# taleinat/fuzzysearch

Hardware: NVIDIA H100
Metric: haystack_GB_per_s_scanned (higher is better)
Workload: dtype u8

## Files before the change

### fuzzysearch_b200/csrc/api.cu

```cuda
#include <algorithm>
#include <atomic>
#include <cstdarg>
#include <cstdio>
#include <cmath>
#include <cstring>
#include <dlfcn.h>
#include <sched.h>
#include <unistd.h>
#include <condition_variable>
#include <memory>
#include <mutex>
#include <thread>
#include <new>
#include <string>
#include <type_traits>
#include <vector>

#include "kernels.cuh"
#include "ham_kernels.cuh"
#include "lp_kernels.cuh"
#include "post_kernels.cuh"
#include "p2p_kernels.cuh"
#include "batch_kernels.cuh"
#include "ham_batch_kernels.cuh"
#include "generic_batch_kernels.cuh"
#include "best_kernels.cuh"
#include "nearest_kernels.cuh"
#include "sym_kernels.cuh"
#include "align_kernels.cuh"
#include <unordered_map>
#include "debug_kernels.cuh"

using namespace fzb;

static thread_local std::string g_err;

static int fail(int code, const char *fmt, ...) {
    char buf[512];
    va_list ap;
    va_start(ap, fmt);
    vsnprintf(buf, sizeof buf, fmt, ap);
    va_end(ap);
    g_err = buf;
    return code;
// ... 54 lines not shown
    T *p_ = nullptr;
    uint64_t n_ = 0;
};
template <class T> using DevBuf = Buf<T, Mem::Device>;
template <class T> using PinnedBuf = Buf<T, Mem::Pinned>;
template <class T> using MappedBuf = Buf<T, Mem::Mapped>;

struct BatchBufs {
    DevBuf<uint32_t> d_mbits;
    DevBuf<uint2> d_gtab;
    DevBuf<uint32_t> d_postings, d_pinfo;
    DevBuf<BatchPat> d_bpats;
    DevBuf<unsigned long long> d_mset;
    DevBuf<WorkItem> d_mwork;
};
struct LpBatchBufs {
    DevBuf<ulonglong2> d_lmlut;
    DevBuf<unsigned long long> d_lmlist;
    DevBuf<unsigned long long> d_lmkept;
    DevBuf<uint32_t> d_lmhist;
};
struct GenericBatchBufs {
    DevBuf<uint32_t> d_glim;
};
struct PeerBufs {
    DevBuf<uint8_t> d_p2p;
    DevBuf<MergeScratch> d_ms;
    DevBuf<unsigned long long> d_mscore;
    DevBuf<uint32_t> d_mpos;
    MappedBuf<int64_t> h_grows;
    MappedBuf<uint32_t> h_ghdr;
};
struct RecBufs {
    DevBuf<uint64_t> d_off;
    DevBuf<uint32_t> d_first;
    uint64_t longest = 0;
};
struct BestBufs {
    DevBuf<uint64_t> d_words;
    DevBuf<uint32_t> d_ids;
};
struct BestState {
    uint64_t *best, *top2;
    const uint32_t *ordinal;
};
struct NearBufs {
// ... 108 lines not shown
    uint32_t p2p_cap = 4096;
    uint64_t slot_bytes = 0, flags_off = 0;
    uint32_t epoch = 0;
    bool counters_clean = false;
    uint32_t seq = 0;
    void *comm = nullptr;
    int rank = 0, world = 1;
    uint32_t gather_cap = 4096;
    std::unique_ptr<GatherBufs> gather;
    cudaEvent_t ev[4] = {nullptr, nullptr, nullptr, nullptr};
    int sm_count = 132;
    DevBuf<uint64_t> d_hits;
    DevBuf<uint32_t> d_glist;
    uint32_t glist_cap = 0;
    DevBuf<uint32_t> d_scratch;
    DevBuf<unsigned long long> d_lplist;
    std::unique_ptr<BatchBufs> batch;
    DevBuf<unsigned long long> d_mhits;
    std::unique_ptr<LpBatchBufs> lpb;
    std::unique_ptr<GenericBatchBufs> gbatch;
    std::unique_ptr<RecBufs> recs;
    std::unique_ptr<BestBufs> bestb;
    std::unique_ptr<NearBufs> nearb;
};

struct fzb_result {
    std::vector<RawRec> raw;
    uint32_t raw_n = 0;
    fzb_haystack *owner = nullptr;
    bool raw_in_stage = false;
    void fetch_raw();
    void discard_attempt();
    std::vector<RawRec> fin;
    std::vector<int64_t> hulls;
    bool unconsolidated = false;
    bool have_fin = false;
    bool device_post = false;
    bool raw_ordered = false;
    bool has_global = false;
    bool global_on_device = false;
    bool fused_issued = false;
    uint32_t fused_status = 0;
    uint32_t gcount = 0;
    std::vector<RawRec> gfin;
    int raw_order = 0;
    void order_raw();
    fzb_stats stats{};
};

static uint64_t round_up(uint64_t x, uint64_t a) { return (x + a - 1) / a * a; }

static RawRec make_rec(int64_t start, int64_t end, int64_t dist) {
    RawRec r;
    r.start = start;
// ... 5 lines not shown
}

struct HandleLock {
    std::recursive_mutex *m;
    explicit HandleLock(fzb_haystack *h) : m(h ? &h->mu : nullptr) {
        if (m) m->lock();
    }
    ~HandleLock() {
        if (m) m->unlock();
    }
    HandleLock(const HandleLock &) = delete;
    HandleLock &operator=(const HandleLock &) = delete;
};

static std::mutex g_pending_mutex;

void fzb_result::fetch_raw() {
    std::lock_guard<std::mutex> lock(g_pending_mutex);
    if (!owner) return;
    if (raw_in_stage) {
        raw.resize(raw_n);
        if (raw_n) {
            cudaSetDevice(owner->device);
            if (cudaMemcpyAsync(raw.data(), owner->d_out.get(), (size_t)raw_n * sizeof(RawRec), cudaMemcpyDeviceToHost,
                                owner->stream) != cudaSuccess ||
                cudaStreamSynchronize(owner->stream) != cudaSuccess) {
                cudaGetLastError();
                raw.clear();
                raw_n = 0;
            }
        }
        raw_in_stage = false;
    }
    if (global_on_device) {
        gfin.resize(gcount);
        for (uint32_t i = 0; i < gcount; i++) {
            const int64_t s0 = owner->peer->h_grows[2 * (size_t)i], v = owner->peer->h_grows[2 * (size_t)i + 1];
            gfin[i] = make_rec(s0, s0 + (v >> 32), v & 0xFFFFFFFF);
        }
        global_on_device = false;
    }
    owner->pending = nullptr;
    owner = nullptr;
}

void fzb_result::discard_attempt() {
    fetch_raw();
    raw.clear();
    raw_n = 0;
    fin.clear();
}

static void detach_pending(fzb_haystack *h) {
    fzb_result *r;
    {
        std::lock_guard<std::mutex> lock(g_pending_mutex);
        r = h->pending;
    }
    if (r) r->fetch_raw();
}

static int alloc_out(fzb_haystack *h, uint64_t cap) { return h->d_out.alloc(cap, cap * (sizeof(RawRec) + sizeof(uint64_t))); }

static int haystack_common_init(fzb_haystack *h) {
    CK(cudaSetDevice(h->device));
    CK(cudaStreamCreateWithFlags(&h->stream, cudaStreamNonBlocking));
    for (auto &e : h->ev) CK(cudaEventCreate(&e));
    CK(cudaEventCreate(&h->ev_stop));
    cudaDeviceProp prop;
    CK(cudaGetDeviceProperties(&prop, h->device));
    h->sm_count = prop.multiProcessorCount;
    uint64_t granules = (h->padded_len >> kGranuleShift) + 2;
    TRY(h->d_bitmap.alloc(round_up((granules + 31) / 32, 32)));
    TRY(h->d_counters.alloc(CNT_COUNT));
    TRY(h->h_counters.alloc(CNT_COUNT));
    memset(h->h_counters.get(), 0, CNT_COUNT * sizeof(uint32_t));
    TRY(h->h_fin.alloc((uint64_t)kPostMax * kFinCols));
    TRY(h->d_fin.alloc((uint64_t)kPostMax * kFinCols));
    TRY(h->d_sorted.alloc(kPostMax));
    CK(cudaFuncSetAttribute(k_post, cudaFuncAttributeMaxDynamicSharedMemorySize, (int)kPostSmem));
    CK(cudaMemset(h->d_bitmap.get(), 0, h->d_bitmap.size() * sizeof(uint32_t)));
    h->glist_cap = (uint32_t)std::min<uint64_t>(granules, 1u << 20);
    TRY(h->d_glist.alloc(std::max<uint32_t>(h->glist_cap, 1)));
    return alloc_out(h, 1u << 16);
}

static int check_shard(uint64_t buf_len, uint64_t buf_lo, uint64_t global_len, uint64_t own_lo,
                       uint64_t own_hi) {
    if (global_len >= (1ull << 46)) return fail(FZB_E_INVALID, "global_len must be below 2^46");
    if (buf_lo > global_len || buf_len > global_len - buf_lo || own_lo > own_hi || own_hi > global_len ||
        (own_lo < own_hi && (own_lo < buf_lo || own_hi > buf_lo + buf_len)))
        return fail(FZB_E_INVALID, "inconsistent shard geometry");
    if (buf_lo % 16 != 0) return fail(FZB_E_INVALID, "buf_lo must be a multiple of 16");
    if (buf_len >= (1ull << 40)) return fail(FZB_E_INVALID, "buf_len must be below 2^40");
    return FZB_OK;
}

static int alloc_buffer(fzb_haystack *h) {
    CK(cudaSetDevice(h->device));
    TRY(h->owned_buf.alloc(h->padded_len));
    h->d = h->owned_buf.get();
    CK(cudaMemset(h->d + h->buf_len, 0, h->padded_len - h->buf_len));
    return FZB_OK;
}

static void close_peers(fzb_haystack *h);
static int upload_bytes(fzb_haystack *h, uint64_t dst_off, const uint8_t *host, uint64_t n);

extern "C" void fzb_haystack_destroy(fzb_haystack *h) {
    if (!h) return;
    cudaSetDevice(h->device);
    if (h->stream) cudaStreamSynchronize(h->stream);
    detach_pending(h);
    if (h->comm) nccl_comm_destroy(h->comm);
    close_peers(h);
    for (auto &e : h->ev)
        if (e) cudaEventDestroy(e);
    if (h->ev_stop) cudaEventDestroy(h->ev_stop);
    if (h->stream) cudaStreamDestroy(h->stream);
    delete h;
}

static int haystack_new(const char *arg_error, const uint8_t *host, const void *dev_ptr, uint64_t buf_len,
                        uint64_t buf_lo, uint64_t global_len, uint64_t own_lo, uint64_t own_hi, int device,
                        fzb_haystack **out) {
    if (!out) return fail(FZB_E_INVALID, "out is NULL");
    *out = nullptr;
    if (arg_error) return fail(FZB_E_INVALID, "%s", arg_error);
    int rc = check_shard(buf_len, buf_lo, global_len, own_lo, own_hi);
    if (rc) return rc;
    if (fzb_device_count() <= device || device < 0)
        return fail(FZB_E_CUDA, "CUDA device %d not available (%d devices)", device, fzb_device_count());
    fzb_haystack *h = new (std::nothrow) fzb_haystack();
    if (!h) return fail(FZB_E_CUDA, "out of host memory");
    h->device = device;
    h->d = (uint8_t *)dev_ptr;
// ... 1454 lines not shown
        TRY(b.d_bpats.alloc(kMaxBatchPats));
        TRY(b.d_mset.alloc(1u << 22));
        CK(cudaMemset(b.d_mset.get(), 0, b.d_mset.size() * sizeof(unsigned long long)));
        TRY(b.d_mwork.alloc(1u << 21));
        CK(cudaFuncSetAttribute(k_filter_multi, cudaFuncAttributeMaxDynamicSharedMemorySize, (int)kMultiSmem));
        return FZB_OK;
    });
}

static int read_counters(fzb_haystack *h, uint32_t cnts[CNT_COUNT]) {
    CK(cudaMemcpyAsync(cnts, h->d_counters.get(), CNT_COUNT * sizeof(uint32_t), cudaMemcpyDeviceToHost, h->stream));
    CK(cudaStreamSynchronize(h->stream));
    return FZB_OK;
}

static void add_stats(fzb_stats *sum, const fzb_stats &s) {
    sum->gpu_ms += s.gpu_ms;
    sum->filter_ms += s.filter_ms;
    sum->bytes_scanned += s.bytes_scanned;
    sum->n_candidates += s.n_candidates;
    sum->n_launches += s.n_launches;
}

static int split_batch(const std::vector<RawRec> &raw, const std::vector<uint32_t> &ids, const fzb_stats &pass,
                       int raw_order, bool unconsolidated, fzb_result **out, fzb_stats *sum) {
    const uint32_t cnt = (uint32_t)ids.size();
    std::vector<uint32_t> per(cnt, 0);
    for (const RawRec &r : raw) per[(uint32_t)r.ngram >> 8]++;
    for (uint32_t i = 0; i < cnt; i++) {
        fzb_result *res = new (std::nothrow) fzb_result();
        if (!res) return fail(FZB_E_CUDA, "out of host memory");
        res->raw.reserve(per[i]);
        if (i == 0) res->stats = pass;
        res->stats.route = pass.route;
        res->raw_order = raw_order;
        out[ids[i]] = res;
    }
    for (const RawRec &r : raw) {
        RawRec q = r;
        q.ngram = r.ngram & 0xFF;
        out[ids[(uint32_t)r.ngram >> 8]]->raw.push_back(q);
    }
    const unsigned nthreads = std::min<unsigned>({8u, std::max(1u, std::thread::hardware_concurrency()), cnt});
    std::atomic<uint32_t> next{0};
    auto work = [&]() {
        for (uint32_t i = next.fetch_add(1); i < cnt; i = next.fetch_add(1)) {
            fzb_result *res = out[ids[i]];
            res->raw_n = (uint32_t)res->raw.size();
            res->unconsolidated = unconsolidated;
            if (unconsolidated)
                finalize_on_host(res, 2);
            else
                consolidate_recs(res->raw, res->fin, &res->hulls);
            res->have_fin = true;
        }
    };
    std::vector<std::thread> pool;
    for (unsigned t = 1; t < nthreads; t++) pool.emplace_back(work);
    work();
    for (auto &t : pool) t.join();
    add_stats(sum, pass);
    return FZB_OK;
}

static int best_accumulate(fzb_haystack *h, const BestState &best, uint32_t n, const uint32_t *d_ids, uint32_t id) {
    if (n == 0) return FZB_OK;
    const int grid = (int)std::min<uint32_t>((n + kBestThreads - 1) / kBestThreads, (uint32_t)h->sm_count * 8);
    if (d_ids)
        k_best_accumulate<true><<<grid, kBestThreads, 0, h->stream>>>(h->d_out.get(), n, rec_set(h), d_ids, id,
                                                                     best.best, best.top2);
    else
        k_best_accumulate<false><<<grid, kBestThreads, 0, h->stream>>>(h->d_out.get(), n, rec_set(h), d_ids, id,
                                                                      best.best, best.top2);
    CK(cudaGetLastError());
    return FZB_OK;
}

struct BatchCall {
    fzb_haystack *h;
    const uint8_t *patterns;
    const uint32_t *offsets;
    uint32_t count, flags;
    std::vector<Plan> plans;
    fzb_result **out;
    const BestState *best;
    std::vector<uint8_t> done;
    bool tiny, share;
    fzb_stats sum{};

    BatchCall(fzb_haystack *h_, const uint8_t *p, const uint32_t *o, uint32_t n, uint32_t f, fzb_result **out_,
              const BestState *best_)
        : h(h_), patterns(p), offsets(o), count(n), flags(f), out(out_), best(best_), done(best_ ? n : 0, 0),
          tiny((f & FZB_F_TINY_LIST) != 0), share((f & ~(FZB_F_TINY_LIST | FZB_F_PER_RECORD)) == 0 && h_->buf_len > 0) {}

    uint32_t len(uint32_t i) const { return offsets[i + 1] - offsets[i]; }
    bool settled(uint32_t i) const { return best ? done[i] != 0 : out[i] != nullptr; }

    template <class P>
    int begin(P plan) {
        for (uint32_t i = 0; i < count; i++) out[i] = nullptr;
        TRY(check_batch_records(h, flags));
        for (uint32_t i = 0; i < count; i++)
            if (offsets[i + 1] < offsets[i]) return fail(FZB_E_INVALID, "offsets must be non-decreasing");
        plans.resize(count);
        for (uint32_t i = 0; i < count; i++) TRY(plan(i, patterns + offsets[i], len(i), plans[i]));
        return FZB_OK;
    }

    int settle(int rc, const std::vector<uint32_t> &ids) {
        auto drop = [&](uint32_t j) {
            if (!out) return;
            fzb_result_destroy(out[j]);
            out[j] = nullptr;
        };
        if (rc < 0)
            for (uint32_t j = 0; j < count; j++) drop(j);
        if (rc > 0)
            for (uint32_t id : ids) drop(id);
        return rc < 0 ? rc : FZB_OK;
    }

    int finish_pass(const std::vector<RawRec> &raw, uint32_t n, const std::vector<uint32_t> &ids, fzb_stats pass,
                    int raw_order, bool unconsolidated) {
        if (!best) return split_batch(raw, ids, pass, raw_order, unconsolidated, out, &sum);
        if (n) {
            std::vector<uint32_t> ordinals(ids.size());
            for (size_t j = 0; j < ids.size(); j++) ordinals[j] = best->ordinal[ids[j]];
            CK(cudaMemcpyAsync(h->bestb->d_ids.get(), ordinals.data(), ordinals.size() * sizeof(uint32_t),
                               cudaMemcpyHostToDevice, h->stream));
            TRY(best_accumulate(h, *best, n, h->bestb->d_ids.get(), 0));
            pass.n_launches++;
        }
        for (uint32_t id : ids) done[id] = 1;
        add_stats(&sum, pass);
        return FZB_OK;
    }

    int finish(fzb_stats *total) {
        const uint32_t f = (flags & ~FZB_F_PER_RECORD) | (best ? FZB_F_NO_FINAL : 0u);
        for (uint32_t i = 0; i < count; i++) {
            if (settled(i)) continue;
            fzb_result *res = nullptr;
            auto planned = [&](Plan &pl) { pl = plans[i]; return FZB_OK; };
            TRY(settle(run_search(h, patterns + offsets[i], f, &res, planned), {}));
            if (!best) {
                add_stats(&sum, res->stats);
                out[i] = res;
                continue;
            }
            const int rc = best_accumulate(h, *best, res->raw_n, nullptr, best->ordinal[i]);
            if (res->raw_n) res->stats.n_launches++;
            add_stats(&sum, res->stats);
            fzb_result_destroy(res);
            TRY(rc);
        }
        sum.route = 7;
        if (total) *total = sum;
        return FZB_OK;
    }
};

template <class F>
static int run_batch_pass(const BatchCall &c, F enqueue, std::vector<RawRec> &raw, uint32_t cnts[CNT_COUNT],
                          fzb_stats &pass) {
    fzb_haystack *h = c.h;
    detach_pending(h);
    for (int attempt = 0; attempt < 8; attempt++) {
        h->counters_clean = false;
        CK(cudaMemsetAsync(h->d_counters.get(), 0, CNT_COUNT * sizeof(uint32_t), h->stream));
        CK(cudaEventRecord(h->ev[0], h->stream));
        int rc = enqueue();
        if (rc) return rc;
        CK(cudaEventRecord(h->ev[2], h->stream));
        rc = read_counters(h, cnts);
        if (rc) return rc;
        if (cnts[CNT_OVERFLOW]) return 1;
        const uint32_t n = cnts[CNT_OUT];
        if (n > kMaxRawRecs) return 1;
        if (n > h->d_out.size()) {
            TRY(ensure_out_cap(h, n));
            continue;
        }
        if (!c.best) raw.resize(n);
        if (!raw.empty()) {
            CK(cudaMemcpyAsync(raw.data(), h->d_out.get(), (size_t)n * sizeof(RawRec), cudaMemcpyDeviceToHost, h->stream));
            CK(cudaStreamSynchronize(h->stream));
        }
        float ms = 0.f;
        cudaEventElapsedTime(&ms, h->ev[0], h->ev[2]);
        pass.gpu_ms = ms;
        pass.bytes_scanned = h->buf_len;
        return FZB_OK;
    }
    return fail(FZB_E_CUDA, "output buffer kept overflowing");
}

struct ChunkSums {
    float scan_ms = 0.f;
    uint64_t listed = 0;
    uint32_t chunks = 0;
};

template <class S, class V>
static int run_chunks(fzb_haystack *h, uint64_t chunk, int list, int full, uint32_t cnts[CNT_COUNT], ChunkSums &s,
                      S scan, V verify) {
    s = ChunkSums{};
    for (uint64_t lo = h->own_lo; lo < h->own_hi; lo += chunk) {
        CK(cudaMemsetAsync(h->d_counters.get() + list, 0, 2 * sizeof(uint32_t), h->stream));
        CK(cudaEventRecord(h->ev[1], h->stream));
// ... 136 lines not shown
    std::vector<uint32_t> bits(kMultiTblWords + (dense ? 0 : kMulti2Words), 0);
    int rc = upload_pass_tables(h, grams, bits, pinfo, pats, [&](uint32_t w) {
        const uint32_t hb = (w * kHashMul) >> (32 - kMultiTblBits);
        bits[hb >> 5] |= 1u << (hb & 31u);
        if (!dense) {
            const uint32_t h2 = multi_hash2(w);
            bits[kMultiTblWords + (h2 >> 5)] |= 1u << (h2 & 31u);
        }
    });
    if (rc) return rc;
    if (dense) TRY(ensure_mhits(h));
    const int ggrid = h->sm_count * 4;
    if (generic) TRY(prepare_generic_pass(c, ids, ggrid));
    BatchBufs &b = *h->batch;
    MultiParams mp = pass_params(h);
    mp.bits2 = dense ? nullptr : b.d_mbits.get() + kMultiTblWords;
    mp.set = b.d_mset.get();
    mp.set_mask = (uint32_t)b.d_mset.size() - 1;
    mp.work = b.d_mwork.get();
    mp.work_cap = c.tiny ? std::min<uint32_t>(b.d_mwork.size(), kTinyBatchCap) : (uint32_t)b.d_mwork.size();
    const uint32_t hits_cap = c.tiny ? std::min<uint32_t>(h->d_mhits.size(), kTinyBatchCap) : (uint32_t)h->d_mhits.size();
    const int64_t nvec = (int64_t)(round_up(h->buf_len, 16) / 16);
    const int64_t ntiles = (nvec + kMultiTileVecs - 1) / kMultiTileVecs;
    std::vector<RawRec> raw;
    uint32_t cnts[CNT_COUNT];
    fzb_stats pass{};
    const RecSet rs = rec_set(h);
    rc = run_batch_pass(c, [&]() -> int {
        MdenseParams dp{mp, b.d_bpats.get(), h->d_mhits.get(), hits_cap};
        if (ntiles > 0) {
            const int grid = (int)std::min<int64_t>(ntiles, h->sm_count);
            if (dense)
                k_filter_mdense<<<grid, kMultiThreads, kMdenseSmem, h->stream>>>(dp, nvec, ntiles);
            else
                k_filter_multi<<<grid, kMultiThreads, kMultiSmem, h->stream>>>(mp, nvec, ntiles);
        }
        CK(cudaEventRecord(h->ev[1], h->stream));
        with_recs(h, [&](auto rec) {
            constexpr bool R = decltype(rec)::value;
            if (generic && dense)
                k_verify_mhits_generic<R><<<ggrid, kLpThreads, 0, h->stream>>>(
                    dp, h->gbatch->d_glim.get(), h->d_scratch.get(), kGenericBatchCap, h->d_out.get(), h->d_out.size(),
                    h->d_counters.get(), rs);
            else if (generic)
                k_verify_multi_generic<R><<<ggrid, kLpThreads, 0, h->stream>>>(
                    mp, b.d_bpats.get(), h->gbatch->d_glim.get(), h->d_scratch.get(), kGenericBatchCap, h->d_out.get(),
                    h->d_out.size(), h->d_counters.get(), rs);
            else if (dense)
                k_verify_mhits<R><<<h->sm_count * 8, kMhThreads, 0, h->stream>>>(dp, h->d_out.get(), h->d_out.size(),
                                                                                    h->d_counters.get(), rs);
            else
                k_verify_multi<R><<<h->sm_count * 8, kVmThreads, 0, h->stream>>>(
                    mp, b.d_bpats.get(), h->d_out.get(), h->d_out.size(), h->d_counters.get(), rs);
        });
        CK(cudaGetLastError());
        return FZB_OK;
    }, raw, cnts, pass);
    if (rc > 0 && !dense) {
        CK(cudaMemsetAsync(b.d_mset.get(), 0, b.d_mset.size() * sizeof(unsigned long long), h->stream));
        CK(cudaStreamSynchronize(h->stream));
    }
    if (rc) return rc;
    float filter_ms = 0.f;
    cudaEventElapsedTime(&filter_ms, h->ev[0], h->ev[1]);
    pass.route = generic ? 9 : dense ? 2 : 1;
    pass.filter_ms = filter_ms;
    pass.n_candidates = cnts[CNT_CAND];
    pass.n_launches = 2;
    return c.finish_pass(raw, cnts[CNT_OUT], ids, pass, generic ? 2 : 0, false);
}

static int batch_pass_lp(BatchCall &c, const std::vector<uint32_t> &ids) {
    fzb_haystack *h = c.h;
    const uint32_t cnt = (uint32_t)ids.size();
    const bool generic = c.plans[ids[0]].generic();
    std::vector<BatchPat> pats(cnt);
    std::vector<ulonglong2> lut(256, make_ulonglong2(0ull, 0ull));
    std::vector<uint32_t> pm32((size_t)cnt * 256, 0u);
    LpMultiParams lp{};
    int wmax = 0;
    uint32_t kmax = 0;
    for (uint32_t i = 0; i < cnt; i++) {
        const uint32_t id = ids[i], m = c.len(id), k = c.plans[id].k;
        BatchPat &bp = pats[i];
        fill_pat(bp, c, id);
        for (uint32_t j = 0; j < m; j++) {
            lut[bp.P[j]].x |= 1ull << i;
            pm32[(size_t)i * 256 + bp.P[j]] |= 1u << j;
        }
        if (generic)
            for (int c = 0; c < 256; c++) lut[c].y |= 1ull << i;
        else
// ... 19 lines not shown
    uint32_t *d_pm32 = reinterpret_cast<uint32_t *>(lb.d_lmlut.get() + 256);
    CK(cudaMemcpyAsync(d_pm32, pm32.data(), pm32.size() * sizeof(uint32_t), cudaMemcpyHostToDevice, h->stream));
    CK(cudaMemcpyAsync(h->batch->d_bpats.get(), pats.data(), pats.size() * sizeof(BatchPat), cudaMemcpyHostToDevice, h->stream));
    lp.H = h->d;
    lp.buf_lo = (int64_t)h->buf_lo;
    lp.buf_len = (int64_t)h->buf_len;
    lp.N = (int64_t)h->global_len;
    lp.lut = lb.d_lmlut.get();
    lp.wmax = wmax;
    lp.pats = h->batch->d_bpats.get();
    lp.pm32 = d_pm32;
    lp.list = lb.d_lmlist.get();
    lp.list_cap = c.tiny ? std::min<uint32_t>(lb.d_lmlist.size(), kTinyLpListCap) : (uint32_t)lb.d_lmlist.size();
    lp.counters = h->d_counters.get();
    int per_sm = 2;
    CK(cudaOccupancyMaxActiveBlocksPerMultiprocessor(&per_sm, k_lp_scan_multi, kLmThreads, kLmSmem));
    per_sm = std::max(per_sm, 1);
    const int vgrid = h->sm_count * 4, sim_cap = 256;
    if (generic)
        TRY(prepare_generic_pass(c, ids, vgrid));
    else
        TRY(ensure_scratch(h, (uint64_t)vgrid * kLpThreads * 2 * sim_cap));
    const uint64_t chunk = c.tiny ? kTinyLpChunk : 256ull << 20;
    std::vector<RawRec> raw;
    uint32_t cnts[CNT_COUNT];
    fzb_stats pass{};
    const RecSet rs = rec_set(h);
    ChunkSums cs;
    int rc = run_batch_pass(c, [&]() -> int {
        return run_chunks(h, chunk, CNT_LMLIST, CNT_LMWORK, cnts, cs, [&](uint64_t lo, uint64_t hi) {
            lp.own_lo = (int64_t)lo;
            lp.own_hi = (int64_t)hi;
            k_lp_scan_multi<<<h->sm_count * per_sm, kLmThreads, kLmSmem, h->stream>>>(lp);
        }, [&]() -> int {
            CK(cudaMemsetAsync(h->d_counters.get() + CNT_LMNEXT, 0, sizeof(uint32_t), h->stream));
            CK(cudaMemsetAsync(lb.d_lmhist.get(), 0, 256 * sizeof(uint32_t), h->stream));
            k_lm_refine<<<h->sm_count * 8, kLmSortThreads, 0, h->stream>>>(lp, lb.d_lmkept.get(), lb.d_lmhist.get());
            k_lm_scatter<<<h->sm_count * 8, kLmSortThreads, 0, h->stream>>>(lb.d_lmkept.get(), lb.d_lmhist.get(),
                                                                              lb.d_lmhist.get() + 128, lb.d_lmlist.get());
            with_recs(h, [&](auto rec) {
                constexpr bool R = decltype(rec)::value;
                if (generic)
                    k_lp_verify_multi_generic<R><<<vgrid, kLpThreads, 0, h->stream>>>(
                        lp, h->gbatch->d_glim.get(), lb.d_lmlist.get(), lb.d_lmhist.get(), h->d_scratch.get(),
                        kGenericBatchCap, h->d_out.get(), h->d_out.size(), h->d_counters.get(), rs);
                else if (kmax <= 4)
                    k_lp_verify_multi<4, R><<<vgrid, kLpThreads, 0, h->stream>>>(
                        lp, lb.d_lmlist.get(), lb.d_lmhist.get(), h->d_scratch.get(), sim_cap, h->d_out.get(),
                        h->d_out.size(), h->d_counters.get(), rs);
                else
                    k_lp_verify_multi<8, R><<<vgrid, kLpThreads, 0, h->stream>>>(
                        lp, lb.d_lmlist.get(), lb.d_lmhist.get(), h->d_scratch.get(), sim_cap, h->d_out.get(),
                        h->d_out.size(), h->d_counters.get(), rs);
            });
            return FZB_OK;
        });
    }, raw, cnts, pass);
    if (rc) return rc;
    pass.route = generic ? 10 : 3;
    pass.filter_ms = cs.scan_ms;
    pass.n_candidates = cs.listed;
    pass.n_launches = 4 * cs.chunks;
    return c.finish_pass(raw, cnts[CNT_OUT], ids, pass, 1, false);
}

constexpr double kDnaLevPostNs = 0.53;
constexpr double kDnaLevHitNs = 0.31;
constexpr double kDnaLevAloneMs = 0.13;
constexpr double kDnaLevAloneReadNs = 4.3e-4;
constexpr double kDnaLevAloneHitNs = 0.29;
constexpr double kDnaLevPassHits = 4.0;
constexpr uint32_t kDnaLevMinL = 5;

static uint32_t dna_lev_postings(const Plan &p) {
    return (p.m / p.L()) << (2 * (kHbKeySyms - std::min<uint32_t>(p.L(), kHbKeySyms)));
}

static double dna_lev_hits(const fzb_haystack *h, const Plan &p, double positions, bool *rides) {
    const uint32_t L = p.L(), n = p.m / L;
    const double c = h->coll_prob;
    const double post = n * std::pow(std::max(c, 0.25), (double)std::min<uint32_t>(L, kHbKeySyms));
    const double hits = n * std::pow(c, (double)L);
    const double pass_ns = positions * (kDnaLevPostNs * post + kDnaLevHitNs * hits);
    const double alone_ns = kDnaLevAloneMs * 1e6 + positions * (kDnaLevAloneReadNs + kDnaLevAloneHitNs * hits);
    *rides = pass_ns < alone_ns;
    return hits;
// ... 7 lines not shown
    Mdense2Params p{};
    two_bit_code(c.patterns, c.offsets, ids, p.code);
    std::unordered_map<uint32_t, std::vector<uint32_t>> keys;
    keys.reserve(cnt * 64);
    for (uint32_t i = 0; i < cnt; i++) {
        const uint32_t id = ids[i], m = c.len(id), k = c.plans[id].k;
        BatchPat &bp = pats[i];
        fill_pat(bp, c, id);
        bp.L = (int)c.plans[id].L();
        bp.n_ngrams = (int)m / bp.L;
        pinfo[i] = m | (k << 8) | ((uint32_t)bp.L << 16);
        for (int j = 0; j < bp.n_ngrams; j++) two_bit_key(keys, p.code, bp.P + j * bp.L, bp.L, (i << 8) | (uint32_t)j);
    }
    std::vector<uint32_t> bits(kHbKeyWords, 0);
    int rc = upload_pass_tables(h, keys, bits, pinfo, pats, [&](uint32_t w) { bits[w >> 5] |= 1u << (w & 31u); });
    if (rc) return rc;
    TRY(ensure_mhits(h));
    const uint32_t hits_cap = c.tiny ? std::min<uint32_t>(h->d_mhits.size(), kTinyBatchCap) : (uint32_t)h->d_mhits.size();
    p.dp = MdenseParams{pass_params(h), h->batch->d_bpats.get(), h->d_mhits.get(), hits_cap};
    const uint64_t tile = (uint64_t)kMultiTileVecs * 16;
    const uint64_t chunk = c.tiny ? kTinyLpChunk
                                  : std::max(tile, (uint64_t)(hits_cap / 2 / std::max(hits_per_pos, 1e-9)) / tile * tile);
    const int64_t nvec = (int64_t)(round_up(h->buf_len, 16) / 16);
    std::vector<RawRec> raw;
    uint32_t cnts[CNT_COUNT];
    fzb_stats pass{};
    const RecSet rs = rec_set(h);
    ChunkSums cs;
    rc = run_batch_pass(c, [&]() -> int {
        return run_chunks(h, chunk, CNT_MHITS, CNT_OVERFLOW, cnts, cs, [&](uint64_t lo, uint64_t hi) {
            p.scan_lo = (int64_t)lo;
            p.scan_hi = (int64_t)hi;
            const int64_t v0 = (p.scan_lo - (int64_t)h->buf_lo) / 16;
            const int64_t v1 = (p.scan_hi - (int64_t)h->buf_lo + 15) / 16;
            const int64_t ntiles = (v1 - v0 + kMultiTileVecs - 1) / kMultiTileVecs;
            p.dp.mp.counters = h->d_counters.get();
            k_filter_mdense2<<<(int)std::min<int64_t>(ntiles, h->sm_count), kMultiThreads, kMdense2Smem, h->stream>>>(
                p, nvec, v0, ntiles);
        }, [&]() -> int {
            with_recs(h, [&](auto rec) {
                constexpr bool R = decltype(rec)::value;
                k_verify_mhits<R><<<h->sm_count * 8, kMhThreads, 0, h->stream>>>(p.dp, h->d_out.get(), h->d_out.size(),
                                                                                    h->d_counters.get(), rs);
            });
            return FZB_OK;
        });
    }, raw, cnts, pass);
    if (rc) return rc;
    pass.route = 2;
    pass.filter_ms = cs.scan_ms;
    pass.n_candidates = cs.listed;
    pass.n_launches = 2 * cs.chunks;
    return c.finish_pass(raw, cnts[CNT_OUT], ids, pass, 0, false);
}

template <class F>
static int qsample_passes(BatchCall &c, F admit) {
    std::vector<uint32_t> shared;
    for (uint32_t i = 0; i < c.count; i++)
        if (admit(i)) shared.push_back(i);
    size_t done = 0;
    while (done < shared.size()) {
        std::vector<uint32_t> ids;
        uint64_t ngr = 0;
        while (done < shared.size() && ids.size() < kMaxBatchPats) {
            const uint32_t m = c.len(shared[done]);
            if (ngr + (m - 3) > kMaxBatchGrams) break;
            ngr += m - 3;
            ids.push_back(shared[done++]);
        }
        if (ids.size() < 2) break;
        TRY(c.settle(batch_pass(c, ids, false), ids));
    }
    return FZB_OK;
}

// ... 319 lines not shown
        bits[b >> 5] |= 1u << (b & 31u);
        if (!two_bit) {
            const uint32_t h2 = multi_hash2(w);
            bits[kMultiTblWords + (h2 >> 5)] |= 1u << (h2 & 31u);
        }
    });
    if (rc) return rc;
    hp.mp = pass_params(h);
    hp.mp.bits2 = two_bit ? nullptr : h->batch->d_mbits.get() + kMultiTblWords;
    hp.pats = h->batch->d_bpats.get();
    const size_t smem = two_bit ? kHbSmem2 : kMultiSmem;
    const RecSet rs = rec_set(h);
    const void *fn = nullptr;
    with_recs(h, [&](auto rec) {
        constexpr bool R = decltype(rec)::value;
        fn = two_bit ? (const void *)k_ham_batch_scan<true, R> : (const void *)k_ham_batch_scan<false, R>;
    });
    CK(cudaFuncSetAttribute(fn, cudaFuncAttributeMaxDynamicSharedMemorySize, (int)smem));
    int per_sm = 1;
    CK(cudaOccupancyMaxActiveBlocksPerMultiprocessor(&per_sm, fn, kMultiThreads, smem));
    per_sm = std::max(per_sm, 1);
    const int64_t nvec = (int64_t)(round_up(h->buf_len, 16) / 16);
    const int64_t ntiles = (nvec + kMultiTileVecs - 1) / kMultiTileVecs;
    std::vector<RawRec> raw;
    uint32_t cnts[CNT_COUNT];
    fzb_stats pass{};
    rc = run_batch_pass(c, [&]() -> int {
        hp.out = h->d_out.get();
        hp.cap = h->d_out.size();
        if (ntiles > 0) {
            const int grid = (int)std::min<int64_t>(ntiles, (int64_t)h->sm_count * per_sm);
            with_recs(h, [&](auto rec) {
                constexpr bool R = decltype(rec)::value;
                if (two_bit)
                    k_ham_batch_scan<true, R><<<grid, kMultiThreads, smem, h->stream>>>(hp, nvec, ntiles, rs);
                else
                    k_ham_batch_scan<false, R><<<grid, kMultiThreads, smem, h->stream>>>(hp, nvec, ntiles, rs);
            });
        }
        CK(cudaGetLastError());
        return FZB_OK;
    }, raw, cnts, pass);
    if (rc) return rc;
    if (c.tiny && cnts[CNT_OUT] > kTinyBatchCap) return 1;
    pass.route = 8;
    pass.filter_ms = pass.gpu_ms;
    pass.n_candidates = cnts[CNT_CAND];
    pass.n_launches = 1;
    return c.finish_pass(raw, cnts[CNT_OUT], ids, pass, 1, true);
}

static int hamming_batch(BatchCall &c, fzb_stats *total) {
    fzb_haystack *h = c.h;
    if (c.share && c.count >= 2 && sample_collision_prob(h) == FZB_OK) {
        const bool two_bit = h->coll_prob >= 0.15;
        for (uint32_t key = two_bit ? (uint32_t)kHbKeySyms : 4u; key >= (two_bit ? (uint32_t)kHbKeySyms : 3u); key--) {
            std::vector<PassItem> items;
            for (uint32_t i = 0; i < c.count; i++) {
                const Plan &p = c.plans[i];
                if (ham_batch_key(p, two_bit) != key) continue;
                const double cost = ham_batch_cost(h, p, key, two_bit);
                if (cost > kHamBatchPatExpect) continue;
                items.push_back({i, cost, ham_batch_postings(p, two_bit)});
            }
            TRY(greedy_passes(items, kHamBatchExpect, [&](const std::vector<uint32_t> &ids, double) {
                return c.settle(batch_pass_ham(c, ids, two_bit, key), ids);
            }));
        }
    }
    return c.finish(total);
}

// ... 878 lines not shown
    if (which != FZB_RAW && r->has_global) const_cast<fzb_result *>(r)->fetch_raw();
    const std::vector<RawRec> &v = (which != FZB_RAW && r->has_global) ? r->gfin : (which == FZB_RAW ? r->raw : r->fin);
    const bool anchors = (which == FZB_RAW) && (r->stats.route <= 2);
    for (size_t i = 0; i < v.size(); i++) {
        if (start) start[i] = v[i].start;
        if (end) end[i] = v[i].end;
        if (dist) dist[i] = v[i].dist;
        if (anchor_ngram) anchor_ngram[i] = anchors ? v[i].ngram : -1;
        if (anchor_idx) anchor_idx[i] = anchors ? v[i].idx : -1;
    }
    return FZB_OK;
}

extern "C" int fzb_result_stats(const fzb_result *r, fzb_stats *out) {
    if (!r || !out) return fail(FZB_E_INVALID, "NULL argument");
    *out = r->stats;
    return FZB_OK;
}

extern "C" void fzb_result_destroy(fzb_result *r) {
    if (!r) return;
    {
        std::lock_guard<std::mutex> lock(g_pending_mutex);
        if (r->owner) {
            r->owner->pending = nullptr;
            r->owner = nullptr;
        }
    }
    delete r;
}
```

Measured before the change: 2867.

## Move batch result split, sort and consolidation onto the GPU

Replaces host-side splitting and consolidation of batched raw match records with a GPU pipeline. The pipeline histograms matches per pattern, scans, scatters into a staging buffer, sorts keys with chunked bitonic sort plus merge passes, and sweeps them into final rows. Raw records stay on device in the stage buffer and are copied to the host lazily only when requested, which removes the bulk device-to-host copy and the multithreaded host post-processing. In exchange it adds several kernel launches, log-depth merge passes, and more complex staging and lifetime bookkeeping for result objects.

```diff
diff --git a/fuzzysearch_b200/csrc/api.cu b/fuzzysearch_b200/csrc/api.cu
--- a/fuzzysearch_b200/csrc/api.cu
+++ b/fuzzysearch_b200/csrc/api.cu
@@ -20,6 +20,7 @@
 #include "ham_kernels.cuh"
 #include "lp_kernels.cuh"
 #include "post_kernels.cuh"
+#include "batch_post_kernels.cuh"
 #include "p2p_kernels.cuh"
 #include "batch_kernels.cuh"
 #include "ham_batch_kernels.cuh"
@@ -120,6 +121,14 @@
 };
 struct GenericBatchBufs {
     DevBuf<uint32_t> d_glim;
+};
+struct BatchPostBufs {
+    DevBuf<uint32_t> d_seg;
+    MappedBuf<uint32_t> h_meta;
+    DevBuf<uint64_t> d_keys;
+    DevBuf<int64_t> d_rows;
+    PinnedBuf<int64_t> h_rows;
+    uint64_t cap = 0;
 };
 struct PeerBufs {
     DevBuf<uint8_t> d_p2p;
@@ -274,6 +283,10 @@
     std::unique_ptr<RecBufs> recs;
     std::unique_ptr<BestBufs> bestb;
     std::unique_ptr<NearBufs> nearb;
+    BatchPostBufs bpost;
+    DevBuf<RawRec> d_stage;
+    uint64_t stage_used = 0;
+    std::vector<fzb_result *> staged;
 };
 
 struct fzb_result {
@@ -281,7 +294,11 @@
     uint32_t raw_n = 0;
     fzb_haystack *owner = nullptr;
     bool raw_in_stage = false;
+    bool batch_stage = false;
+    uint64_t stage_off = 0;
+    uint32_t stage_slot = 0;
     void fetch_raw();
+    void unlink();
     void discard_attempt();
     std::vector<RawRec> fin;
     std::vector<int64_t> hulls;
@@ -333,7 +350,8 @@
         raw.resize(raw_n);
         if (raw_n) {
             cudaSetDevice(owner->device);
-            if (cudaMemcpyAsync(raw.data(), owner->d_out.get(), (size_t)raw_n * sizeof(RawRec), cudaMemcpyDeviceToHost,
+            const RawRec *src = batch_stage ? owner->d_stage.get() + stage_off : owner->d_out.get();
+            if (cudaMemcpyAsync(raw.data(), src, (size_t)raw_n * sizeof(RawRec), cudaMemcpyDeviceToHost,
                                 owner->stream) != cudaSuccess ||
                 cudaStreamSynchronize(owner->stream) != cudaSuccess) {
                 cudaGetLastError();
@@ -351,8 +369,17 @@
         }
         global_on_device = false;
     }
-    owner->pending = nullptr;
+    unlink();
+}
+
+void fzb_result::unlink() {
+    if (batch_stage)
+        owner->staged[stage_slot] = nullptr;
+    else
+        owner->pending = nullptr;
     owner = nullptr;
+    batch_stage = false;
+    raw_in_stage = false;
 }
 
 void fzb_result::discard_attempt() {
@@ -370,6 +397,34 @@
     }
     if (r) r->fetch_raw();
 }
+
+static void detach_stage(fzb_haystack *h) {
+    std::lock_guard<std::mutex> lock(g_pending_mutex);
+    bool live = false;
+    for (fzb_result *r : h->staged) live |= r != nullptr;
+    if (live) {
+        std::vector<RawRec> all(h->stage_used);
+        cudaSetDevice(h->device);
+        const bool ok = cudaMemcpyAsync(all.data(), h->d_stage.get(), all.size() * sizeof(RawRec), cudaMemcpyDeviceToHost,
+                                        h->stream) == cudaSuccess &&
+                        cudaStreamSynchronize(h->stream) == cudaSuccess;
+        if (!ok) cudaGetLastError();
+        for (fzb_result *r : h->staged) {
+            if (!r) continue;
+            if (ok)
+                r->raw.assign(all.begin() + r->stage_off, all.begin() + r->stage_off + r->raw_n);
+            else {
+                r->raw.clear();
+                r->raw_n = 0;
+            }
+            r->unlink();
+        }
+    }
+    h->staged.clear();
+    h->stage_used = 0;
+}
+
+constexpr uint64_t kBpMinCap = 1u << 12;
 
 static int alloc_out(fzb_haystack *h, uint64_t cap) { return h->d_out.alloc(cap, cap * (sizeof(RawRec) + sizeof(uint64_t))); }
 
@@ -393,6 +448,13 @@
     CK(cudaMemset(h->d_bitmap.get(), 0, h->d_bitmap.size() * sizeof(uint32_t)));
     h->glist_cap = (uint32_t)std::min<uint64_t>(granules, 1u << 20);
     TRY(h->d_glist.alloc(std::max<uint32_t>(h->glist_cap, 1)));
+    TRY(h->bpost.d_seg.alloc(4 * ((uint64_t)kBpMaxPats + 1)));
+    TRY(h->bpost.h_meta.alloc(2 * (uint64_t)kBpMaxPats + 2));
+    TRY(h->bpost.d_keys.alloc(2 * kBpMinCap));
+    TRY(h->bpost.d_rows.alloc(kBpMinCap * kFinCols));
+    TRY(h->bpost.h_rows.alloc(kBpMinCap * kFinCols));
+    h->bpost.cap = kBpMinCap;
+    TRY(h->d_stage.alloc(kBpMinCap));
     return alloc_out(h, 1u << 16);
 }
 
@@ -423,6 +485,7 @@
     cudaSetDevice(h->device);
     if (h->stream) cudaStreamSynchronize(h->stream);
     detach_pending(h);
+    detach_stage(h);
     if (h->comm) nccl_comm_destroy(h->comm);
     close_peers(h);
     for (auto &e : h->ev)
@@ -1923,43 +1986,95 @@
     sum->n_launches += s.n_launches;
 }
 
-static int split_batch(const std::vector<RawRec> &raw, const std::vector<uint32_t> &ids, const fzb_stats &pass,
-                       int raw_order, bool unconsolidated, fzb_result **out, fzb_stats *sum) {
+static_assert(kMaxBatchPats == kBpMaxPats, "batch_post_kernels.cuh sizes its per-pattern tables for kMaxBatchPats");
+
+static int post_batch(fzb_haystack *h, uint32_t n, const std::vector<uint32_t> &ids, fzb_stats pass, int raw_order,
+                      bool unconsolidated, fzb_result **out, fzb_stats *sum) {
     const uint32_t cnt = (uint32_t)ids.size();
-    std::vector<uint32_t> per(cnt, 0);
-    for (const RawRec &r : raw) per[(uint32_t)r.ngram >> 8]++;
+    BatchPostBufs &b = h->bpost;
+    if (n > b.cap) {
+        uint64_t cap = std::max<uint64_t>(b.cap, kBpMinCap);
+        while (cap < n) cap *= 2;
+        TRY(b.d_keys.alloc(2 * cap));
+        TRY(b.d_rows.alloc(cap * kFinCols));
+        TRY(b.h_rows.alloc(cap * kFinCols));
+        b.cap = cap;
+    }
+    if (h->stage_used + n > kMaxRawRecs) detach_stage(h);
+    if (h->stage_used + n > h->d_stage.size()) {
+        uint64_t cap = std::max<uint64_t>(h->d_stage.size(), kBpMinCap);
+        while (cap < h->stage_used + n) cap *= 2;
+        DevBuf<RawRec> grown;
+        TRY(grown.alloc(cap));
+        if (h->stage_used)
+            CK(cudaMemcpyAsync(grown.get(), h->d_stage.get(), h->stage_used * sizeof(RawRec), cudaMemcpyDeviceToDevice,
+                               h->stream));
+        std::lock_guard<std::mutex> lock(g_pending_mutex);
+        h->d_stage = std::move(grown);
+    }
+    uint32_t *hist = b.d_seg.get(), *seg = hist + kBpMaxPats + 1, *cur = seg + kBpMaxPats + 1, *chunk = cur + kBpMaxPats + 1;
+    uint32_t *meta = b.h_meta.get(), *nfin = meta + kBpMaxPats + 2;
+    if (n) {
+        meta[0] = 0;
+        CK(cudaEventRecord(h->ev[1], h->stream));
+        CK(cudaMemsetAsync(hist, 0, cnt * sizeof(uint32_t), h->stream));
+        const int grid = (int)std::min<uint64_t>((n + kBpThreads - 1) / kBpThreads, (uint64_t)h->sm_count * 4);
+        k_bp_count<<<grid, kBpThreads, 0, h->stream>>>(h->d_out.get(), n, cnt, hist);
+        k_bp_scan<<<1, kPostThreads, 0, h->stream>>>(hist, cnt, seg, cur, chunk, meta);
+        uint64_t *keys = b.d_keys.get(), *keys2 = keys + b.cap;
+        k_bp_scatter<<<grid, kBpThreads, 0, h->stream>>>(h->d_out.get(), n, cnt, (int64_t)h->buf_lo, cur,
+                                                         h->d_stage.get() + h->stage_used, keys, meta);
+        const uint32_t chunks = (n + kBpChunk - 1) / kBpChunk + cnt;
+        k_bp_sort_chunks<<<chunks, kBpSortThreads, kBpSortSmem, h->stream>>>(keys, seg, chunk, cnt);
+        const uint64_t per_cta = (uint64_t)kBpMergeItems * kBpThreads;
+        const uint32_t mgrid = (uint32_t)((n + per_cta - 1) / per_cta);
+        for (uint64_t w = kBpChunk; w < n; w *= 2) {
+            k_bp_merge<<<mgrid, kBpThreads, 0, h->stream>>>(keys, keys2, seg, cnt, (uint32_t)w);
+            std::swap(keys, keys2);
+        }
+        k_bp_sweep<<<cnt, kPostThreads, 0, h->stream>>>(keys, seg, (int64_t)h->buf_lo, unconsolidated ? 2 : 1,
+                                                        b.d_rows.get(), nfin);
+        CK(cudaGetLastError());
+        CK(cudaMemcpyAsync(b.h_rows.get(), b.d_rows.get(), (size_t)n * kFinCols * sizeof(int64_t), cudaMemcpyDeviceToHost,
+                           h->stream));
+        CK(cudaEventRecord(h->ev[2], h->stream));
+        CK(cudaStreamSynchronize(h->stream));
+        float ms = 0.f;
+        cudaEventElapsedTime(&ms, h->ev[1], h->ev[2]);
+        pass.gpu_ms += ms;
+        if (meta[0]) return fail(FZB_E_UNSUPPORTED, "a batch match lies outside the bounds of its canonical key");
+    }
     for (uint32_t i = 0; i < cnt; i++) {
         fzb_result *res = new (std::nothrow) fzb_result();
         if (!res) return fail(FZB_E_CUDA, "out of host memory");
-        res->raw.reserve(per[i]);
+        out[ids[i]] = res;
         if (i == 0) res->stats = pass;
         res->stats.route = pass.route;
         res->raw_order = raw_order;
-        out[ids[i]] = res;
-    }
-    for (const RawRec &r : raw) {
-        RawRec q = r;
-        q.ngram = r.ngram & 0xFF;
-        out[ids[(uint32_t)r.ngram >> 8]]->raw.push_back(q);
-    }
-    const unsigned nthreads = std::min<unsigned>({8u, std::max(1u, std::thread::hardware_concurrency()), cnt});
-    std::atomic<uint32_t> next{0};
-    auto work = [&]() {
-        for (uint32_t i = next.fetch_add(1); i < cnt; i = next.fetch_add(1)) {
-            fzb_result *res = out[ids[i]];
-            res->raw_n = (uint32_t)res->raw.size();
-            res->unconsolidated = unconsolidated;
-            if (unconsolidated)
-                finalize_on_host(res, 2);
-            else
-                consolidate_recs(res->raw, res->fin, &res->hulls);
-            res->have_fin = true;
-        }
-    };
-    std::vector<std::thread> pool;
-    for (unsigned t = 1; t < nthreads; t++) pool.emplace_back(work);
-    work();
-    for (auto &t : pool) t.join();
+        res->unconsolidated = unconsolidated;
+        const uint32_t lo = n ? meta[1 + i] : 0, nf = n ? nfin[i] : 0;
+        res->raw_n = n ? meta[2 + i] - lo : 0;
+        res->fin.resize(nf);
+        res->hulls.resize((size_t)nf * 2);
+        for (uint32_t g = 0; g < nf; g++) {
+            const int64_t *row = b.h_rows.get() + (size_t)kFinCols * (lo + g);
+            res->fin[g] = make_rec(row[0], row[1], row[2]);
+            res->hulls[2 * (size_t)g] = row[3];
+            res->hulls[2 * (size_t)g + 1] = row[4];
+        }
+        res->have_fin = true;
+        res->device_post = true;
+        if (res->raw_n) {
+            std::lock_guard<std::mutex> lock(g_pending_mutex);
+            res->owner = h;
+            res->raw_in_stage = true;
+            res->batch_stage = true;
+            res->stage_off = h->stage_used + lo;
+            res->stage_slot = (uint32_t)h->staged.size();
+            h->staged.push_back(res);
+        }
+    }
+    h->stage_used += n;
     add_stats(sum, pass);
     return FZB_OK;
 }
@@ -2000,6 +2115,7 @@
     template <class P>
     int begin(P plan) {
         for (uint32_t i = 0; i < count; i++) out[i] = nullptr;
+        if (out) detach_stage(h);
         TRY(check_batch_records(h, flags));
         for (uint32_t i = 0; i < count; i++)
             if (offsets[i + 1] < offsets[i]) return fail(FZB_E_INVALID, "offsets must be non-decreasing");
@@ -2021,9 +2137,8 @@
         return rc < 0 ? rc : FZB_OK;
     }
 
-    int finish_pass(const std::vector<RawRec> &raw, uint32_t n, const std::vector<uint32_t> &ids, fzb_stats pass,
-                    int raw_order, bool unconsolidated) {
-        if (!best) return split_batch(raw, ids, pass, raw_order, unconsolidated, out, &sum);
+    int finish_pass(uint32_t n, const std::vector<uint32_t> &ids, fzb_stats pass, int raw_order, bool unconsolidated) {
+        if (!best) return post_batch(h, n, ids, pass, raw_order, unconsolidated, out, &sum);
         if (n) {
             std::vector<uint32_t> ordinals(ids.size());
             for (size_t j = 0; j < ids.size(); j++) ordinals[j] = best->ordinal[ids[j]];
@@ -2062,8 +2177,7 @@
 };
 
 template <class F>
-static int run_batch_pass(const BatchCall &c, F enqueue, std::vector<RawRec> &raw, uint32_t cnts[CNT_COUNT],
-                          fzb_stats &pass) {
+static int run_batch_pass(const BatchCall &c, F enqueue, uint32_t cnts[CNT_COUNT], fzb_stats &pass) {
     fzb_haystack *h = c.h;
     detach_pending(h);
     for (int attempt = 0; attempt < 8; attempt++) {
@@ -2081,11 +2195,6 @@
         if (n > h->d_out.size()) {
             TRY(ensure_out_cap(h, n));
             continue;
-        }
-        if (!c.best) raw.resize(n);
-        if (!raw.empty()) {
-            CK(cudaMemcpyAsync(raw.data(), h->d_out.get(), (size_t)n * sizeof(RawRec), cudaMemcpyDeviceToHost, h->stream));
-            CK(cudaStreamSynchronize(h->stream));
         }
         float ms = 0.f;
         cudaEventElapsedTime(&ms, h->ev[0], h->ev[2]);
@@ -2268,7 +2377,6 @@
     const uint32_t hits_cap = c.tiny ? std::min<uint32_t>(h->d_mhits.size(), kTinyBatchCap) : (uint32_t)h->d_mhits.size();
     const int64_t nvec = (int64_t)(round_up(h->buf_len, 16) / 16);
     const int64_t ntiles = (nvec + kMultiTileVecs - 1) / kMultiTileVecs;
-    std::vector<RawRec> raw;
     uint32_t cnts[CNT_COUNT];
     fzb_stats pass{};
     const RecSet rs = rec_set(h);
@@ -2301,7 +2409,7 @@
         });
         CK(cudaGetLastError());
         return FZB_OK;
-    }, raw, cnts, pass);
+    }, cnts, pass);
     if (rc > 0 && !dense) {
         CK(cudaMemsetAsync(b.d_mset.get(), 0, b.d_mset.size() * sizeof(unsigned long long), h->stream));
         CK(cudaStreamSynchronize(h->stream));
@@ -2313,7 +2421,7 @@
     pass.filter_ms = filter_ms;
     pass.n_candidates = cnts[CNT_CAND];
     pass.n_launches = 2;
-    return c.finish_pass(raw, cnts[CNT_OUT], ids, pass, generic ? 2 : 0, false);
+    return c.finish_pass(cnts[CNT_OUT], ids, pass, generic ? 2 : 0, false);
 }
 
 static int batch_pass_lp(BatchCall &c, const std::vector<uint32_t> &ids) {
@@ -2379,7 +2487,6 @@
     else
         TRY(ensure_scratch(h, (uint64_t)vgrid * kLpThreads * 2 * sim_cap));
     const uint64_t chunk = c.tiny ? kTinyLpChunk : 256ull << 20;
-    std::vector<RawRec> raw;
     uint32_t cnts[CNT_COUNT];
     fzb_stats pass{};
     const RecSet rs = rec_set(h);
@@ -2412,13 +2519,13 @@
             });
             return FZB_OK;
         });
-    }, raw, cnts, pass);
+    }, cnts, pass);
     if (rc) return rc;
     pass.route = generic ? 10 : 3;
     pass.filter_ms = cs.scan_ms;
     pass.n_candidates = cs.listed;
     pass.n_launches = 4 * cs.chunks;
-    return c.finish_pass(raw, cnts[CNT_OUT], ids, pass, 1, false);
+    return c.finish_pass(cnts[CNT_OUT], ids, pass, 1, false);
 }
 
 constexpr double kDnaLevPostNs = 0.53;
@@ -2472,7 +2579,6 @@
     const uint64_t chunk = c.tiny ? kTinyLpChunk
                                   : std::max(tile, (uint64_t)(hits_cap / 2 / std::max(hits_per_pos, 1e-9)) / tile * tile);
     const int64_t nvec = (int64_t)(round_up(h->buf_len, 16) / 16);
-    std::vector<RawRec> raw;
     uint32_t cnts[CNT_COUNT];
     fzb_stats pass{};
     const RecSet rs = rec_set(h);
@@ -2495,13 +2601,13 @@
             });
             return FZB_OK;
         });
-    }, raw, cnts, pass);
+    }, cnts, pass);
     if (rc) return rc;
     pass.route = 2;
     pass.filter_ms = cs.scan_ms;
     pass.n_candidates = cs.listed;
     pass.n_launches = 2 * cs.chunks;
-    return c.finish_pass(raw, cnts[CNT_OUT], ids, pass, 0, false);
+    return c.finish_pass(cnts[CNT_OUT], ids, pass, 0, false);
 }
 
 template <class F>
@@ -2867,7 +2973,6 @@
     per_sm = std::max(per_sm, 1);
     const int64_t nvec = (int64_t)(round_up(h->buf_len, 16) / 16);
     const int64_t ntiles = (nvec + kMultiTileVecs - 1) / kMultiTileVecs;
-    std::vector<RawRec> raw;
     uint32_t cnts[CNT_COUNT];
     fzb_stats pass{};
     rc = run_batch_pass(c, [&]() -> int {
@@ -2885,14 +2990,14 @@
         }
         CK(cudaGetLastError());
         return FZB_OK;
-    }, raw, cnts, pass);
+    }, cnts, pass);
     if (rc) return rc;
     if (c.tiny && cnts[CNT_OUT] > kTinyBatchCap) return 1;
     pass.route = 8;
     pass.filter_ms = pass.gpu_ms;
     pass.n_candidates = cnts[CNT_CAND];
     pass.n_launches = 1;
-    return c.finish_pass(raw, cnts[CNT_OUT], ids, pass, 1, true);
+    return c.finish_pass(cnts[CNT_OUT], ids, pass, 1, true);
 }
 
 static int hamming_batch(BatchCall &c, fzb_stats *total) {
@@ -3817,10 +3922,7 @@
     if (!r) return;
     {
         std::lock_guard<std::mutex> lock(g_pending_mutex);
-        if (r->owner) {
-            r->owner->pending = nullptr;
-            r->owner = nullptr;
-        }
+        if (r->owner) r->unlink();
     }
     delete r;
 }
diff --git a/fuzzysearch_b200/csrc/batch_post_kernels.cuh b/fuzzysearch_b200/csrc/batch_post_kernels.cuh
--- /dev/null
+++ b/fuzzysearch_b200/csrc/batch_post_kernels.cuh
@@ -0,0 +1,228 @@
+#pragma once
+#include "post_kernels.cuh"
+
+namespace fzb {
+
+constexpr uint32_t kBpMaxPats = 4096;
+constexpr int kBpThreads = 256;
+constexpr int kBpChunk = 4096;
+constexpr int kBpSortThreads = 1024;
+constexpr size_t kBpSortSmem = (size_t)kBpChunk * 8;
+static_assert(kBpSortSmem <= 48 * 1024, "k_bp_sort_chunks runs without a dynamic shared-memory opt-in");
+constexpr uint32_t kBpMergeItems = 8;
+constexpr uint64_t kBpPosMask = (1ull << 46) - 1;
+
+__device__ __forceinline__ uint64_t bp_min(uint64_t a, uint64_t b) { return a < b ? a : b; }
+__device__ __forceinline__ uint32_t bp_slice(uint32_t n, uint32_t b, uint32_t G) { return (uint32_t)((uint64_t)n * b / G); }
+
+__global__ void __launch_bounds__(kBpThreads)
+k_bp_count(const RawRec *raw, uint32_t n, uint32_t cnt, uint32_t *hist) {
+    __shared__ uint32_t s_h[kBpMaxPats];
+    for (uint32_t p = threadIdx.x; p < cnt; p += kBpThreads) s_h[p] = 0;
+    __syncthreads();
+    const uint32_t lo = bp_slice(n, blockIdx.x, gridDim.x), hi = bp_slice(n, blockIdx.x + 1, gridDim.x);
+    for (uint32_t i = lo + threadIdx.x; i < hi; i += kBpThreads) {
+        const uint32_t p = (uint32_t)raw[i].ngram >> 8;
+        if (p < cnt) atomicAdd(&s_h[p], 1u);
+    }
+    __syncthreads();
+    for (uint32_t p = threadIdx.x; p < cnt; p += kBpThreads)
+        if (s_h[p]) atomicAdd(&hist[p], s_h[p]);
+}
+
+__global__ void __launch_bounds__(kPostThreads, 1)
+k_bp_scan(const uint32_t *hist, uint32_t cnt, uint32_t *seg, uint32_t *cur, uint32_t *chunk, uint32_t *meta) {
+    __shared__ uint32_t scr[33];
+    uint32_t carry = 0, carry_chunks = 0;
+    for (uint32_t base = 0; base < cnt; base += kPostThreads) {
+        const uint32_t p = base + threadIdx.x;
+        const uint32_t c = p < cnt ? hist[p] : 0u;
+        uint32_t total, total_chunks;
+        const uint32_t off = carry + block_scan_sum(c, scr, &total);
+        const uint32_t coff = carry_chunks + block_scan_sum((c + kBpChunk - 1) / kBpChunk, scr, &total_chunks);
+        if (p < cnt) {
+            seg[p] = off;
+            cur[p] = off;
+            chunk[p] = coff;
+            meta[1 + p] = off;
+        }
+        carry += total;
+        carry_chunks += total_chunks;
+    }
+    if (threadIdx.x == 0) {
+        seg[cnt] = carry;
+        chunk[cnt] = carry_chunks;
+        meta[1 + cnt] = carry;
+    }
+}
+
+__global__ void __launch_bounds__(kBpThreads)
+k_bp_scatter(const RawRec *raw, uint32_t n, uint32_t cnt, int64_t buf_lo, uint32_t *cur, RawRec *stage, uint64_t *keys,
+             uint32_t *meta) {
+    __shared__ uint32_t s_h[kBpMaxPats];
+    for (uint32_t p = threadIdx.x; p < cnt; p += kBpThreads) s_h[p] = 0;
+    __syncthreads();
+    const uint32_t lo = bp_slice(n, blockIdx.x, gridDim.x), hi = bp_slice(n, blockIdx.x + 1, gridDim.x);
+    for (uint32_t i = lo + threadIdx.x; i < hi; i += kBpThreads) {
+        const uint32_t p = (uint32_t)raw[i].ngram >> 8;
+        if (p < cnt) atomicAdd(&s_h[p], 1u);
+    }
+    __syncthreads();
+    for (uint32_t p = threadIdx.x; p < cnt; p += kBpThreads)
+        if (s_h[p]) s_h[p] = atomicAdd(&cur[p], s_h[p]);
+    __syncthreads();
+    for (uint32_t i = lo + threadIdx.x; i < hi; i += kBpThreads) {
+        RawRec r = raw[i];
+        const uint32_t p = (uint32_t)r.ngram >> 8;
+        const int64_t rel = r.start - buf_lo, len = r.end - r.start;
+        if (p >= cnt || rel < 0 || rel > (int64_t)kBpPosMask || len < 0 || len > 1023 || r.dist < 0 || r.dist > 255) {
+            meta[0] = 1u;
+            continue;
+        }
+        const uint32_t pos = atomicAdd(&s_h[p], 1u);
+        r.ngram &= 0xFF;
+        stage[pos] = r;
+        keys[pos] = ((uint64_t)rel << 18) | ((uint64_t)len << 8) | (uint64_t)r.dist;
+    }
+}
+
+__device__ __forceinline__ uint32_t bp_find(const uint32_t *v, uint32_t cnt, uint32_t o) {
+    uint32_t lo = 0, hi = cnt;
+    while (hi - lo > 1) {
+        const uint32_t mid = (lo + hi) / 2;
+        if (v[mid] <= o) lo = mid; else hi = mid;
+    }
+    return lo;
+}
+
+__global__ void __launch_bounds__(kBpSortThreads)
+k_bp_sort_chunks(uint64_t *keys, const uint32_t *seg, const uint32_t *chunk, uint32_t cnt) {
+    extern __shared__ __align__(16) uint8_t bp_smem[];
+    uint64_t *s = reinterpret_cast<uint64_t *>(bp_smem);
+    const uint32_t c = blockIdx.x;
+    if (c >= chunk[cnt]) return;
+    const uint32_t p = bp_find(chunk, cnt, c);
+    const uint32_t lo = seg[p] + (c - chunk[p]) * (uint32_t)kBpChunk;
+    const uint32_t len = min(seg[p + 1] - lo, (uint32_t)kBpChunk);
+    uint32_t L = 2;
+    while (L < len) L <<= 1;
+    for (uint32_t i = threadIdx.x; i < L; i += kBpSortThreads) s[i] = i < len ? keys[lo + i] : ~0ull;
+    __syncthreads();
+    for (uint32_t k = 2; k <= L; k <<= 1) {
+        for (uint32_t j = k >> 1; j > 0; j >>= 1) {
+            for (uint32_t i = threadIdx.x; i < L; i += kBpSortThreads) {
+                const uint32_t x = i ^ j;
+                if (x > i) {
+                    const uint64_t a = s[i], b = s[x];
+                    if ((a > b) == ((i & k) == 0)) {
+                        s[i] = b;
+                        s[x] = a;
+                    }
+                }
+            }
+            __syncthreads();
+        }
+    }
+    for (uint32_t i = threadIdx.x; i < len; i += kBpSortThreads) keys[lo + i] = s[i];
+}
+
+__global__ void __launch_bounds__(kBpThreads)
+k_bp_merge(const uint64_t *src, uint64_t *dst, const uint32_t *seg, uint32_t cnt, uint32_t width) {
+    const uint32_t n = seg[cnt];
+    const uint64_t t = (uint64_t)blockIdx.x * kBpThreads + threadIdx.x;
+    if (t * kBpMergeItems >= n) return;
+    uint32_t o = (uint32_t)(t * kBpMergeItems);
+    const uint32_t o1 = (uint32_t)bp_min((uint64_t)o + kBpMergeItems, n);
+    while (o < o1) {
+        const uint32_t p = bp_find(seg, cnt, o);
+        const uint32_t base = seg[p], segn = seg[p + 1] - base, rel = o - base;
+        const uint64_t pair = (uint64_t)rel / (2ull * width) * (2ull * width);
+        const uint32_t a_lo = (uint32_t)pair;
+        const uint32_t a_hi = (uint32_t)bp_min(pair + width, segn);
+        const uint32_t b_hi = (uint32_t)bp_min(pair + 2ull * width, segn);
+        const uint64_t *A = src + base + a_lo, *B = src + base + a_hi;
+        const uint32_t la = a_hi - a_lo, lb = b_hi - a_hi;
+        uint32_t k = rel - a_lo;
+        const uint32_t k_end = min(k + (o1 - o), la + lb);
+        uint32_t lo = k > lb ? k - lb : 0u, hi = min(k, la);
+        while (lo < hi) {
+            const uint32_t mid = (lo + hi) / 2;
+            if (A[mid] <= B[k - mid - 1]) lo = mid + 1; else hi = mid;
+        }
+        uint32_t i = lo, j = k - lo;
+        uint64_t *out = dst + base + a_lo;
+        for (; k < k_end; k++) {
+            if (j >= lb || (i < la && A[i] <= B[j])) out[k] = A[i++];
+            else out[k] = B[j++];
+        }
+        o = base + a_lo + k_end;
+    }
+}
+
+__global__ void __launch_bounds__(kPostThreads, 1)
+k_bp_sweep(const uint64_t *keys, const uint32_t *seg, int64_t buf_lo, int mode, int64_t *rows, uint32_t *nfin) {
+    __shared__ unsigned long long s_best[kPostThreads + 1];
+    __shared__ long long s_hs[kPostThreads + 1];
+    __shared__ unsigned long long scr64[33];
+    __shared__ uint32_t scr32[33];
+    const uint32_t p = blockIdx.x, tid = threadIdx.x, lo = seg[p], n = seg[p + 1] - lo;
+    int64_t *prow = rows + (size_t)kFinCols * lo;
+    if (mode == 2) {
+        for (uint32_t i = tid; i < n; i += kPostThreads) {
+            const uint64_t kx = keys[lo + i];
+            const int64_t s = buf_lo + (int64_t)(kx >> 18), e = s + (int64_t)((kx >> 8) & 1023u);
+            int64_t *row = prow + (size_t)kFinCols * i;
+            row[0] = s;
+            row[1] = e;
+            row[2] = (int64_t)(kx & 255u);
+            row[3] = s;
+            row[4] = e;
+        }
+        if (tid == 0) nfin[p] = n;
+        return;
+    }
+    auto write_row = [&](uint32_t g, unsigned long long best, long long hs, unsigned long long he) {
+        const uint64_t kx = keys[lo + (best & kBpPosMask)];
+        const int64_t s = buf_lo + (int64_t)(kx >> 18);
+        int64_t *row = prow + (size_t)kFinCols * g;
+        row[0] = s;
+        row[1] = s + (int64_t)((kx >> 8) & 1023u);
+        row[2] = (int64_t)(kx & 255u);
+        row[3] = buf_lo + hs;
+        row[4] = buf_lo + (int64_t)he;
+    };
+    if (tid == 0) s_best[0] = ~0ull;
+    unsigned long long carry_hull = 0;
+    uint32_t carry_groups = 0;
+    for (uint32_t base = 0; base < n; base += kPostThreads) {
+        const uint32_t i = base + tid;
+        const bool live = i < n;
+        const uint64_t kx = live ? keys[lo + i] : 0;
+        const unsigned long long s = kx >> 18, len = (kx >> 8) & 1023u, e = live ? s + len : 0;
+        unsigned long long round_max;
+        const unsigned long long hull = max(carry_hull, block_scan_max(e, scr64, &round_max));
+        const bool head = live && (i == 0 || s >= hull);
+        uint32_t round_heads;
+        const uint32_t local = block_scan_sum(head ? 1u : 0u, scr32, &round_heads) + (head ? 1u : 0u);
+        s_best[tid + 1] = ~0ull;
+        if (head) s_hs[local] = (long long)s;
+        __syncthreads();
+        if (live) atomicMin(&s_best[local], ((kx & 255u) << 56) | ((1023ull - len) << 46) | (unsigned long long)i);
+        __syncthreads();
+        if (head && carry_groups + local >= 2) write_row(carry_groups + local - 2, s_best[local - 1], s_hs[local - 1], hull);
+        __syncthreads();
+        if (tid == 0) {
+            s_best[0] = s_best[round_heads];
+            s_hs[0] = s_hs[round_heads];
+        }
+        carry_hull = max(carry_hull, round_max);
+        carry_groups += round_heads;
+        __syncthreads();
+    }
+    if (tid == 0) {
+        if (n) write_row(carry_groups - 1, s_best[0], s_hs[0], carry_hull);
+        nfin[p] = carry_groups;
+    }
+}
+
+}
```

Result: no change. 2868 (median of 6 runs) (+0.0%).
